# BUTSpeechFIT/huggingface_asr

Measured on AMD Instinct MI355X. Metric: audio-seconds/sec encoder fwd+CTC, E-Branchformer-base, higher is better.
Workload: dtype bf16; 1 GPU; E-Branchformer-base enc+CTC (relative-pos), 32x10s 16kHz clips/GPU: fbank+CMVN -> conv2d sub -> 16 layers -> CTC head -> CTC loss (the batch-independent projection of the relative-position table, 0.2 % of the FLOPs, is cached across steps); per_gpu_batch=32, frames=1000, encoder_frames=250, parallelism=replicas x1 (no exchange step), steps_in_flight=4, wide_tiles=True, hw_queues=8

## Files before the change

### huggingface_asr_amd/_lib.py

```python
from __future__ import annotations

import ctypes as C
import os

_HERE = os.path.dirname(os.path.abspath(__file__))
LIB_PATH = os.environ.get("HFASR_HIP_LIB") or os.path.join(_HERE, "libhfasr_hip.so")

vp, i32, i64, f32, f64, sz = C.c_void_p, C.c_int, C.c_long, C.c_float, C.c_double, C.c_size_t


class EbfConfig(C.Structure):
    _fields_ = [(n, i32) for n in ("B", "T", "F", "d", "H", "I", "L", "V", "C1", "C2", "K", "stride", "pad",
                                   "is_causal", "pos_type", "csgu_kernel", "merge_kernel", "csgu_act", "use_macaron")] + \
               [("ln_eps", f32), ("logits_f32", i32), ("logits_ld", i32), ("branch_overlap", i32), ("extra_layers", i32), ("layer_mixing", i32), ("csgu_linear", i32),
                ("context_mode", i32), ("gate_blk", i32), ("ln_fold", i32), ("wide_tiles", i32)]


class LnRedDesc(C.Structure):
    _fields_ = [("partial", vp), ("nblk", i32), ("d", i32), ("dgamma", vp), ("dbeta", vp), ("kind", i32)]


class Gpt2Config(C.Structure):
    _fields_ = [("d", i32), ("H", i32), ("L", i32), ("V", i32), ("eps", f32), ("step_form", i32), ("act", i32)]


GLOBAL_SLOTS, LAYER_SLOTS = 24, 64

SIGNATURES = {
    "mi_gemm_bf16": [vp, i64, vp, i64, vp, i32, vp, i64, i32, vp, i64, f32, i32, i32, i32, i32, i32, i32, vp],
    "mi_conv2d_cl_bf16": [vp, vp, vp, vp] + [i32] * 13 + [vp],
    "mi_gemm_bf16_v": [vp, i64, vp, i64, vp, i32, vp, i64, i32, vp, i64, f32, i32, i32, i32, i32, i32, i32, i32, vp],
    "mi_conv2d_cl_bf16_v": [vp, vp, vp, vp] + [i32] * 14 + [vp],
    "mi_conv2d_first_gelu": [vp, vp, vp, vp] + [i32] * 10 + [vp],
    "mi_conv2d_first_geo": [vp, vp, vp, vp] + [i32] * 13 + [vp],
    "mi_conv2d_first_gated_gelu": [vp, vp, vp, vp, vp, vp] + [i32] * 10 + [vp],
    "mi_conv2d_cl_geo_bf16": [vp, vp, vp, vp] + [i32] * 15 + [vp],
    "mi_gated_act_bf16": [vp, i64, vp, i64, vp, i64, i32, i32, i32, i32, i32, i32, vp],
    "mi_im2col_cl_geo_bf16": [vp, vp] + [i32] * 12 + [vp],
    "mi_col2im_cl_bf16": [vp, vp] + [i32] * 13 + [vp],
    "mi_gated_act_bwd_bf16": [vp, i64, vp, i64, vp, i64, vp, i64, vp, i64, i32, i32, i32, i32, i32, vp],
    "mi_conv2d_first_wgrad": [vp, vp, vp, vp] + [i32] * 12 + [vp, vp],
    "mi_gemm_lnfold_bf16": [vp, i64, vp, i64, vp, vp, vp, i32, f32, vp, i64, i32, i32, i32, i32, vp],
    "mi_gemm_resid_stats_f32": [vp, i64, vp, i64, vp, vp, i64, vp, i64, f32, vp, i64, vp, i32, i32, i32, vp],
    "mi_layernorm_fold": [vp, i64, vp, i32, vp, vp, f32, vp, i64, vp, i64, vp, i32, i32, vp],
    "mi_layernorm_chain": [vp, i64, vp, i32, vp, vp, f32, vp, i64, vp, vp, f32, vp, i64, vp, i64, vp, vp, vp, i64, i32, i32, vp],
    "mi_cast_f32_bf16": [vp, i64, vp, i64, i32, i32, vp],
    "mi_rotary_bf16": [vp, i64, vp, i64, vp, vp, i32, i32, i32, i32, vp],
    "mi_attention_bf16": [vp, i64, vp, i64, vp, i64, i32, vp, i64, vp, vp, vp, vp, i64, i32, i32, i32, i32, f32, i32, vp],
    "mi_attention_qkv_bf16": [vp, i64, vp, i64, vp, i64, vp, i64, vp, vp, vp, vp, i64, i32, i32, i32, i64, i32, i32, f32, i32, vp],
    "mi_attention_qkv_bf16_v": [vp, i64, vp, i64, vp, i64, vp, i64, vp, vp, vp, vp, i64, i32, i32, i32, i64, i32, i32, f32, i32, i32, vp],
    "mi_attention_x_lse_bf16": [vp, i64, vp, i64, vp, i64, vp, vp, i64, vp, i32, i32, i32, i32, i32, f32, i32, f32, C.c_uint, C.c_uint, vp],
    "mi_attention_x_bwd_probs": [vp, i64, vp, i64, vp, i64, vp, vp, i64, vp, i64, vp, vp, vp, i64, vp, i64, i32, i32, i32, i32, i32, f32, i32, f32, C.c_uint, C.c_uint, vp],
    "mi_attention_qkv_lse_bf16": [vp, i64, vp, i64, vp, i64, vp, i64, vp, vp, vp, vp, i64, vp, i32, i32, i32, i32, f32, i32, f32, C.c_uint, C.c_uint, vp],
    "mi_attention_qkv_bwd_probs": [vp, i64, vp, i64, vp, i64, vp, i64, vp, vp, vp, vp, i64, vp, i64, vp, vp, vp, i64, vp, i64, i32,
                                   vp, i64, vp, vp, vp, vp, i64, i32, i32, i32, i32, f32, i32, f32, C.c_uint, C.c_uint, i32, vp],
    "mi_attention_qkv_bwd_fused": [vp, vp, vp, i64, vp, vp, i64, vp, i64, vp, vp, vp, vp, i64, vp, sz, i32, i32, i32, i32, f32, vp],
    "mi_row_stats_bf16": [vp, i64, i32, f32, vp, i32, vp],
    "mi_csgu_bf16": [vp, i64, vp, vp, vp, vp, vp, vp, i64, i32, i32, i32, i32, i32, i32, i32, vp],
    "mi_dwconv_residual_bf16": [vp, i64, vp, vp, vp, i64, i32, i32, i32, i32, i32, vp],
    "mi_fbank_f64": [vp, i64, vp, i32, vp, vp, vp, vp, vp, vp, i32, i32, i32, f64, f64, vp],
    "mi_trim_zeros_pad_f32": [vp, i64, vp, i32, i32, i32, vp, i64, i32, vp, vp, vp, vp],
    "mi_cmvn_utterance": [vp, vp, i32, i32, i32, i32, i32, f32, vp],
    "mi_cmvn_global": [vp, i64, i32, vp, vp, vp],
    "mi_row_lse": [vp, i64, i32, i32, vp, i32, vp],
    "mi_gemm_lse_f32": [vp, i64, vp, i64, vp, vp, i64, vp, vp, i32, i32, i32, vp],
    "mi_gemm_lse_workspace_floats": [i32, i32],
    "mi_row_argmax": [vp, i64, i32, i32, vp, i32, vp],
# ... 191 lines not shown
```

### huggingface_asr_amd/csrc/encoder.hip

```cpp
#include "ebf_layout.hpp"

namespace {

struct Ws {
    bf16_t *act1, *act2, *a0, *a1, *a2, *a1r, *h, *qk, *vt, *ctx, *cat, *m2, *s, *hid;
    bf16_t *cv, *lin;
    bf16_t *z1, *g1, *z2, *g2;
    float *feo, *x, *stats, *lnst;
    float *mixed, *lh, *sw;
    int* lens;
    size_t bytes;
};

Ws carve(const mi_ebf_config& c, const Dims& d, void* base) {
    Carver k{(char*)base, 0};
    auto bf = [&](size_t n) { return (bf16_t*)k.take(n * 2); };
    auto f32 = [&](size_t n) { return (float*)k.take(n * 4); };
    Ws w;
    const size_t M = d.M, dd = c.d, I = c.I, n1 = (size_t)c.B * d.T1 * d.F1 * c.C1, n2 = (size_t)c.B * d.T2 * d.F2 * c.C2;
    w.act1 = bf(n1); w.act2 = bf(n2);
    w.z1 = w.g1 = w.z2 = w.g2 = nullptr;
    if (c.context_mode == 1) {
        if (!conv1_gated_fused(c.B, d.T1, d.F1, c.C1, c.K)) { w.z1 = bf(n1); w.g1 = bf(n1); }
        w.z2 = bf(2 * n2);
// ... 207 lines not shown
                                  w.hid, d, nullptr, 0, nullptr, nullptr, nullptr, 0, M, d, st);
    if (c.use_macaron)
        return mi_layernorm_chain(w.x, d, nullptr, T2, Lf(l, FIN_LN_G), Lf(l, FIN_LN_B), LEPS, w.x, d,
                                  Lf(l + 1, FF1_LN_G), Lf(l + 1, FF1_LN_B), LEPS, w.a0, d, nullptr, 0, nullptr, nullptr, nullptr, 0, M, d, st);
    return mi_layernorm_chain(w.x, d, nullptr, T2, Lf(l, FIN_LN_G), Lf(l, FIN_LN_B), LEPS, w.x, d,
                              Lf(l + 1, ATT_LN_G), Lf(l + 1, ATT_LN_B), LEPS, w.a1, d, nullptr, 0,
                              Lf(l + 1, MLP_LN_G), Lf(l + 1, MLP_LN_B), w.a2, d, M, d, st);
}

int Fwd::folded_layer(int l) const {
    const int gv = c.wide_tiles ? 40 : 0;
    const int npg = c.wide_tiles ? d / 64 : d / 32;
    RUN(mi_gemm_lnfold_bf16(w.a0, d, Lw(l, FF1_WF), d, Lf(l, FF1_SF), Lf(l, FF1_CF), w.lnst, 1, LEPS, w.h, I, 1, M, I, d, st));
    RUN(mi_gemm_resid_stats_f32_v(w.h, I, Lw(l, FF1_W2), I, Lf(l, FF1_B2), w.x, d, w.x, d, 0.5f, w.a0, d, w.lnst, M, d, I, gv, st));
    RUN(mi_gemm_lnfold_bf16(w.a0, d, Lw(l, QKV_WF), d, Lf(l, QKV_SF), Lf(l, QKV_CF), w.lnst, npg, LEPS, w.qk, 3 * d, 0, M, 3 * d, d, st));
    RUN(attention_qkv(l));
    RUN(mi_gemm_bf16_v(w.ctx, d, Lw(l, ATT_WO), d, Lf(l, ATT_BO), 1, w.cat, 2 * d, 0, nullptr, 0, 1.f, 0, M, d, d, 0, 0, gv, st));
    RUN(mi_gemm_lnfold_bf16(w.a0, d, Lw(l, MLP_WF), d, Lf(l, MLP_SF), Lf(l, MLP_CF), w.lnst, npg, LEPS, w.h, I, 1, M, I, d, st));
    RUN(local_gate(l, st));
    RUN(mi_gemm_bf16_v(w.s, I / 2, Lw(l, MLP_W2), I / 2, Lf(l, MLP_B2), 1, w.cat + d, 2 * d, 0, nullptr, 0, 1.f, 0, M, d, I / 2, 0, 0, gv, st));
    RUN(merge_dwconv(l));
    RUN(mi_gemm_resid_stats_f32_v(w.m2, 2 * d, Lw(l, MRG_W), 2 * d, Lf(l, MRG_B), w.x, d, w.x, d, 1.0f, w.a0, d, w.lnst, M, d, 2 * d, gv, st));
    RUN(mi_gemm_lnfold_bf16(w.a0, d, Lw(l, FF2_WF), d, Lf(l, FF2_SF), Lf(l, FF2_CF), w.lnst, npg, LEPS, w.h, I, 1, M, I, d, st));
    RUN(mi_gemm_bf16_v(w.h, I, Lw(l, FF2_W2), I, Lf(l, FF2_B2), 1, w.x, d, 1, w.x, d, 0.5f, 0, M, d, I, 0, 0, gv, st));
    if (l + 1 == c.L) return MI_OK;
    return mi_layernorm_fold(w.x, d, nullptr, T2, Lf(l, FIN_LN_G), Lf(l, FIN_LN_B), LEPS, w.x, d, w.a0, d, w.lnst, M, d, st);
}

int Fwd::encoder_exit(int l, float* last_hidden) const {
    const bool tune = c.layer_mixing || c.extra_layers;
    float* lh = (last_hidden || !tune) ? last_hidden : w.lh;
    RUN(mi_layernorm_chain(w.x, d, nullptr, T2, Lf(l, FIN_LN_G), Lf(l, FIN_LN_B), LEPS, nullptr, 0,
                           Gf(G_ENC_LN_G), Gf(G_ENC_LN_B), c.ln_eps, w.hid, d, lh, d, nullptr, nullptr, nullptr, 0, M, d, st));
    if (!tune) return MI_OK;
    const float* top = lh;
    if (c.layer_mixing) {
        RUN(mi_axpy_dev_f32(w.mixed, lh, (long)M * d, w.sw + c.L, 0, st));
        top = w.mixed;
    }
    return c.extra_layers ? enter_layer(top, c.L) : mi_add2_cast_bf16(top, d, nullptr, 0, w.hid, d, M, d, 1.f, st);
}

int Fwd::ctc_head(void* logits, float* lse, float* lse_workspace, int* best, float* amax_workspace) const {
    if (!best && !logits) return MI_OK;
    const long ldl = c.logits_ld > 0 ? c.logits_ld : c.V + 1;
    int rc = MI_ERR_UNSUPPORTED;
// ... 86 lines not shown
```

### huggingface_asr_amd/csrc/gemm_8p.hip

```cpp
#include "gemm_args.hpp"
#include <type_traits>

#ifndef GEMM_FLOOR
#define GEMM_FLOOR 0
#endif
#ifndef GEMM128_LOADER
#define GEMM128_LOADER 0
#endif

namespace {

typedef __attribute__((address_space(1))) const void* gptr_t;
typedef __attribute__((address_space(3))) void* lptr_t;

constexpr int TB = 256, BK = 64;
constexpr int BUF = 65536, BOFF = 32768;

template <int N>
__device__ __forceinline__ void wait_vm() {
    if constexpr (N >= 0) asm volatile("s_waitcnt vmcnt(%0)" ::"n"(N) : "memory");
}
__device__ __forceinline__ void barrier() {
    __builtin_amdgcn_sched_barrier(0);
    asm volatile("s_barrier" ::: "memory");
// ... 1027 lines not shown
                sm += dpp_f32<0x141, 0xF>(0.f, sm); sq += dpp_f32<0x141, 0xF>(0.f, sq);
                if ((ec & 7) == 0 && m < p.M) *reinterpret_cast<f32x2*>(p.stats_out + (long)m * LN_STATS_STRIDE + (((n0 >> 7) << 2) + (ec >> 3)) * 2) = f32x2{sm, sq};
            }
        }
    } else {
        bf16_t* C = reinterpret_cast<bf16_t*>(p.C);
#pragma unroll
        for (int u = 0; u < 8; ++u) {
            const int row = wave * 16 + u * 2 + er;
            const f32x4 v = *reinterpret_cast<const f32x4*>(smem + row * 512 + ((ec ^ (row & 31)) << 4));
            const int m = m0 + row, n = n0 + ec * 4;
            bf16x4 o = {f2bf(v.x), f2bf(v.y), f2bf(v.z), f2bf(v.w)};
            if (p.drop_p > 0.f) {
                float k4[4];
                mask_keep4(p.drop_key, ((unsigned long long)m * (unsigned)p.N + (unsigned)n) >> 2, p.drop_p, 1.f / (1.f - p.drop_p), k4);
#pragma unroll
                for (int q = 0; q < 4; ++q) o[q] = f2bf(bf2f(o[q]) * k4[q]);
            }
            if (m < p.M) *reinterpret_cast<bf16x4*>(C + (long)m * p.ldc + n) = o;
        }
    }
}

}

bool gemm_8p_supported(const GemmArgs& a, bool conv) {
    if (a.M <= 0 || a.N <= 0 || (a.K % BK) != 0 || a.K < 2 * BK) return false;
    if (a.col_T || a.bias_mode == 2) return false;
    if (a.resid && (!a.out_f32 || (a.N % TB) != 0 || ((uintptr_t)a.resid & 15) || (a.ldr % 4) != 0)) return false;
    if (((uintptr_t)a.A & 15) || ((uintptr_t)a.W & 15) || ((uintptr_t)a.C & 15) || (a.ldw % 8)) return false;
    if (a.out_f32) {
        if (conv || a.act != 0 || (a.ldc % 4) != 0 || a.ldc < ((a.N + 3) & ~3)) return false;
    } else {
        if ((a.N % TB) != 0 || (a.ldc % 8) != 0) return false;
        if (a.bias_mode == 1 && ((uintptr_t)a.bias & 15)) return false;
    }
    if (a.gated && (!conv || a.out_f32 || a.act != 1)) return false;
    if (a.ln_stats) {
        if (conv || a.out_f32 || a.gated || a.act > 1 || a.bias_mode != 1 || !a.ln_colsum || ((uintptr_t)a.ln_colsum & 15) || ((uintptr_t)a.ln_stats & 15)) return false;
        if (!(a.ln_npart == 1 || (a.ln_npart >= 4 && a.ln_npart <= 16 && (a.ln_npart % 4) == 0))) return false;
    }
    if (a.act >= 3) {
        if (conv || a.out_f32 || a.gated || a.ln_stats || a.resid || a.col_T || a.act > 4 || (a.aux_kind != 1 && a.aux_kind != 2) || a.drop_p < 0.f || a.drop_p >= 1.f) return false;
        if (a.act == 3 && (!a.aux || ((uintptr_t)a.aux & 15) || (a.ldaux % 8))) return false;
        if (a.act == 4 && (!a.C2 || ((uintptr_t)a.C2 & 15) || (a.ldc2 % 8))) return false;
    } else if (a.C2 || a.stats_out) {
// ... 52 lines not shown
    if (a.out_f32) {
        const bool attr32 = set_lds_attr(gemm8p_kernel<false, 0, true>, 2 * BUF);
        (void)attr32;
        launch_dense(PF_8P_OUT32, gemm8p_kernel<false, 0, true>, dim3(grid), dim3(512), (size_t)2 * BUF, stream, a);
        return MI_OK;
    }
    if (a.ln_stats) {
        const bool attr_l = set_lds_attr(gemm8p_kernel<false, 0, false, false, true>, 2 * BUF + 2048) && set_lds_attr(gemm8p_kernel<false, 1, false, false, true>, 2 * BUF + 2048);
        (void)attr_l;
        if (a.act) launch_dense(PF_8P_GELU, gemm8p_kernel<false, 1, false, false, true>, dim3(grid), dim3(512), (size_t)2 * BUF + 2048, stream, a);
        else launch_dense(PF_8P, gemm8p_kernel<false, 0, false, false, true>, dim3(grid), dim3(512), (size_t)2 * BUF + 2048, stream, a);
        return MI_OK;
    }
    if (a.gated) {
        const bool attr_g = set_lds_attr(gemm8p_kernel<true, 1, false, true>, 2 * BUF);
        (void)attr_g;
        launch_dense(PF_8P_CONV, gemm8p_kernel<true, 1, false, true>, dim3(grid), dim3(512), (size_t)2 * BUF, stream, a);
        return MI_OK;
    }
    launch_dense(conv ? PF_8P_CONV : (a.act ? PF_8P_GELU : PF_8P), kerns[conv ? 1 : 0][a.act], dim3(grid), dim3(512), (size_t)2 * BUF, stream, a);
    return MI_OK;
}

bool gemm_8p128_supported(const GemmArgs& a) {
    if (a.M <= 0 || a.N <= 0 || (a.N % 128) != 0 || (a.K % BK) != 0 || a.K < 5 * BK) return false;
    if (a.col_T || a.bias_mode == 2) return false;
    if (a.resid && !a.out_f32) return false;
    if (((uintptr_t)a.A & 15) || ((uintptr_t)a.W & 15) || ((uintptr_t)a.C & 15) || (a.lda % 8) || (a.ldw % 8)) return false;
    if (a.out_f32 ? (a.ldc % 4) != 0 : (a.ldc % 8) != 0) return false;
    if (a.resid && (((uintptr_t)a.resid & 15) || (a.ldr % 4) != 0)) return false;
    if (a.bias_mode == 1 && ((uintptr_t)a.bias & 15)) return false;
    if ((long)a.M * a.lda * 2 >= (1l << 32) || (long)a.N * a.ldw * 2 >= (1l << 32)) return false;
    if (a.ln_stats) return false;
    if ((a.C2 || a.stats_out) && (!a.out_f32 || a.N > 512 || (a.K % 128) != 0 || (a.C2 && (((uintptr_t)a.C2 & 7) || (a.ldc2 % 4))) || ((uintptr_t)a.stats_out & 7))) return false;
    return true;
}

int gemm_8p128_launch(const GemmArgs& a, int ring, hipStream_t stream) {
    const bool attr_set = set_lds_attr(gemm8p128_kernel<4>, 4 * B128_BUF);
    (void)attr_set;
    const int grid = cdiv(a.M, 128) * (a.N / 128);
    if (ring == 0) ring = (GEMM128_LOADER == 1 && a.K >= 2048) ? 2 : 3;
    if (ring == 2) {
        const bool attr_l = set_lds_attr(gemm8p128l_kernel, 4 * B128_BUF);
        (void)attr_l;
        launch_dense(PF_8P128, gemm8p128l_kernel, dim3(grid), dim3(512), (size_t)4 * B128_BUF, stream, a);
// ... 12 lines not shown
```

### huggingface_asr_amd/csrc/gemm_args.hpp

```cpp
#pragma once
#include "common.hpp"
#include <hip/hip_ext.h>

struct GemmArgs {
    const bf16_t* A; long lda;
    const bf16_t* W; long ldw;
    const float* bias; int bias_mode;
    void* C; long ldc; int out_f32;
    const float* resid; long ldr; float alpha;
    int act;
    int col_T, col_Tp;
    int M, N, K;
    int variant;
    int Tin, Fin, Cin, Tout, Fout, KW, stride, pad_t, pad_f;
    int stride_f;
    int gated;
    const float* ln_stats; int ln_npart; const float* ln_colsum; float ln_eps;
    bf16_t* C2; long ldc2; float* stats_out;
    const bf16_t* aux; long ldaux; int aux_kind; float drop_p; unsigned long long drop_key;
    float* lse_part; int lse_ld;
    float* amax_part; int amax_ld;
    int ce; const long* ce_labels; float* ce_target; const float* ce_lse; const float* ce_g;
};
constexpr int LN_STATS_STRIDE = 32;

bool gemm_glds_supported(const GemmArgs& a, bool conv);
int gemm_glds_launch(const GemmArgs& a, bool conv, hipStream_t stream);


bool gemm_8p_supported(const GemmArgs& a, bool conv);
int gemm_8p_launch(const GemmArgs& a, bool conv, hipStream_t stream);
bool gemm_8p128_supported(const GemmArgs& a);
int gemm_8p128_launch(const GemmArgs& a, int ring, hipStream_t stream);


extern "C" int mi_profile_take_events(hipEvent_t* start, hipEvent_t* stop, int family);
enum { PF_8P = 0, PF_8P_GELU = 1, PF_8P_CONV = 2, PF_8P_OUT32 = 3, PF_8P128 = 4, PF_GLDS = 5, PF_GENERIC = 6, PF_8P_AMAX = 7, PF_8P_CE = 8, PF_COUNT = 9 };

template <typename F, typename... Args>
inline void launch_dense(int family, F kernel, dim3 grid, dim3 block, size_t lds, hipStream_t stream, Args... args) {
    hipEvent_t e0, e1;
    if (mi_profile_take_events(&e0, &e1, family)) hipExtLaunchKernelGGL(kernel, grid, block, (std::uint32_t)lds, stream, e0, e1, 0, args...);
    else hipLaunchKernelGGL(kernel, grid, block, lds, stream, args...);
}
```

### huggingface_asr_amd/csrc/gemm_bf16.hip

```cpp
#include "gemm_args.hpp"

namespace {

constexpr int BM = 128, BN = 128, BK = 64;
constexpr int NT = 256;

__device__ __forceinline__ int swz(int row, int chunk) { return chunk ^ ((row >> 1) & 7); }

template <bool CONV>
__global__ __launch_bounds__(NT) void gemm_bf16_kernel(GemmArgs p) {
    extern __shared__ __attribute__((aligned(16))) char smem[];
    bf16_t* sA = reinterpret_cast<bf16_t*>(smem);
    bf16_t* sB = sA + 2 * BM * BK;

    const int tid = threadIdx.x;
    const int lane = tid & 63, wave = tid >> 6;
    const int wm = wave >> 1, wn = wave & 1;

    const int ntm = (p.M + BM - 1) / BM, ntn = (p.N + BN - 1) / BN;
    const int nwg = ntm * ntn;
    int bid = blockIdx.x;
    {
        const int q = nwg >> 3, r = nwg & 7, xcd = bid & 7, idx = bid >> 3;
        bid = (xcd < r ? xcd * (q + 1) : r * (q + 1) + (xcd - r) * q) + idx;
// ... 293 lines not shown
                                         void* C2, long ldc2, float* stats_out, int M, int N, int K, int variant, hipStream_t stream);
extern "C" int mi_gemm_resid_stats_f32(const void* A, long lda, const void* W, long ldw, const float* bias, float* C, long ldc, const float* resid, long ldr, float alpha,
                                       void* C2, long ldc2, float* stats_out, int M, int N, int K, hipStream_t stream) {
    return mi_gemm_resid_stats_f32_v(A, lda, W, ldw, bias, C, ldc, resid, ldr, alpha, C2, ldc2, stats_out, M, N, K, 0, stream);
}
extern "C" int mi_gemm_resid_stats_f32_v(const void* A, long lda, const void* W, long ldw, const float* bias, float* C, long ldc, const float* resid, long ldr, float alpha,
                                         void* C2, long ldc2, float* stats_out, int M, int N, int K, int variant, hipStream_t stream) {
    MI_ENTER();
    GemmArgs a{};
    a.A = (const bf16_t*)A; a.lda = lda; a.W = (const bf16_t*)W; a.ldw = ldw; a.bias = bias; a.bias_mode = bias ? 1 : 0;
    a.C = C; a.ldc = ldc; a.out_f32 = 1; a.resid = resid; a.ldr = ldr; a.alpha = alpha; a.act = 0; a.M = M; a.N = N; a.K = K;
    a.C2 = (bf16_t*)C2; a.ldc2 = ldc2; a.stats_out = stats_out;
    if (!A || !W || !C || !resid || (variant != 0 && variant != 40 && variant != 42 && variant != 43)) return MI_ERR_ARG;
    const bool wide = variant == 40;
    if (wide ? !gemm_8p_supported(a, false) : !gemm_8p128_supported(a)) return MI_ERR_UNSUPPORTED;
    const int slot = mi_profile_hook_begin(stream, 2.0 * M * N * K);
    const int rc = wide ? gemm_8p_launch(a, false, stream) : gemm_8p128_launch(a, variant == 42 ? 3 : (variant == 43 ? 2 : 0), stream);
    if (slot >= 0) mi_profile_hook_end(slot, stream);
    if (rc != MI_OK) return rc;
    MI_CHECK_LAUNCH();
    return MI_OK;
}

namespace {
__global__ __launch_bounds__(256) void lse_merge_kernel(const float* __restrict__ part, int ld, int npair, float* __restrict__ lse, int M) {
    const int g = threadIdx.x & 15;
    const int row = blockIdx.x * 16 + (threadIdx.x >> 4);
    const float* pr = part + (long)min(row, M - 1) * ld;
    float mx = -INFINITY;
    for (int t = g; t < npair; t += 16) mx = fmaxf(mx, pr[2 * t]);
    mx = fmaxf(mx, dpp_f32<0xB1, 0xF>(mx, mx)); mx = fmaxf(mx, dpp_f32<0x4E, 0xF>(mx, mx));
    mx = fmaxf(mx, dpp_f32<0x141, 0xF>(mx, mx)); mx = fmaxf(mx, dpp_f32<0x140, 0xF>(mx, mx));
    float s = 0.f;
    for (int t = g; t < npair; t += 16) {
        const f32x2 q = *reinterpret_cast<const f32x2*>(pr + 2 * t);
        if (q.x > -INFINITY) s += q.y * __expf(q.x - mx);
    }
    s += dpp_f32<0xB1, 0xF>(0.f, s); s += dpp_f32<0x4E, 0xF>(0.f, s);
    s += dpp_f32<0x141, 0xF>(0.f, s); s += dpp_f32<0x140, 0xF>(0.f, s);
    if (g == 0 && row < M) lse[row] = mx + __logf(s);
}
}

extern "C" size_t mi_gemm_lse_workspace_floats(int M, int N) { return (size_t)(M > 0 ? M : 0) * 8 * (size_t)((N + 255) / 256); }

extern "C" int mi_gemm_lse_f32(const void* A, long lda, const void* W, long ldw, const float* bias, float* C, long ldc, float* lse, float* workspace,
// ... 129 lines not shown
```

### huggingface_asr_amd/ops.py

```python
from __future__ import annotations

import math

import torch

from . import _lib

BF16 = torch.bfloat16


def _p(t):
    return 0 if t is None else t.data_ptr()


_PINNED_STREAM = None


def _stream():
    return torch.cuda.current_stream().cuda_stream if _PINNED_STREAM is None else _PINNED_STREAM


class pinned_stream:

    def __enter__(self):
# ... 105 lines not shown
    _lib.check(_lib.lib().mi_gated_act_bf16(z2.data_ptr(), z2.stride(0), g2.data_ptr(), g2.stride(0), out.data_ptr(), out.stride(0), B, T, Fq, C, share, blk, _stream()),
               "mi_gated_act_bf16")
    return out


def gemm_lnfold(xb, wf, colsum, cbias, stats, npart, eps=1e-5, act="none", out=None):
    M, K = xb.shape
    N = wf.shape[0]
    if out is None:
        out = torch.empty((M, N), device=xb.device, dtype=BF16)
    _lib.check(_lib.lib().mi_gemm_lnfold_bf16(xb.data_ptr(), xb.stride(0), wf.data_ptr(), wf.stride(0), colsum.data_ptr(), cbias.data_ptr(), stats.data_ptr(), int(npart), float(eps),
                                              out.data_ptr(), out.stride(0), {"none": 0, "gelu": 1}[act], M, N, K, _stream()), "mi_gemm_lnfold_bf16")
    return out


def gemm_resid_stats(a, w, bias, resid, alpha=1.0, wide=False, variant=None):
    M, K = a.shape
    N = w.shape[0]
    c = torch.empty((M, N), device=a.device, dtype=torch.float32)
    c2 = torch.empty((M, N), device=a.device, dtype=BF16)
    st = torch.zeros((M, 32), device=a.device, dtype=torch.float32)
    _lib.check(_lib.lib().mi_gemm_resid_stats_f32_v(a.data_ptr(), a.stride(0), w.data_ptr(), w.stride(0), _p(bias), c.data_ptr(), c.stride(0), _p(resid), resid.stride(0) if resid is not None else 0,
                                                    float(alpha), c2.data_ptr(), c2.stride(0), st.data_ptr(), M, N, K, (40 if wide else 0) if variant is None else int(variant), _stream()), "mi_gemm_resid_stats_f32_v")
    return c, c2, st


def layernorm_fold(x, ln=None, eps=1e-5, lengths=None, T=1):
    M, d = x.shape
    g, b = ln if ln else (None, None)
    y = torch.empty_like(x)
    yb = torch.empty((M, d), device=x.device, dtype=BF16)
    st = torch.zeros((M, 32), device=x.device, dtype=torch.float32)
    _lib.check(_lib.lib().mi_layernorm_fold(x.data_ptr(), x.stride(0), _p(lengths), T, _p(g), _p(b), float(eps), y.data_ptr(), y.stride(0), yb.data_ptr(), yb.stride(0), st.data_ptr(),
                                            M, d, _stream()), "mi_layernorm_fold")
    return y, yb, st


def layernorm_chain(x, *, lengths=None, T=1, ln1=None, eps1=1e-5, store_y=None, lna=None, eps2=1e-5, outa=None,
                    outa32=None, lnb=None, outb=None):
    M, d = x.shape
    g1, b1 = ln1 if ln1 else (None, None)
    ga, ba = lna if lna else (None, None)
    gb, bb = lnb if lnb else (None, None)
    rc = _lib.lib().mi_layernorm_chain(x.data_ptr(), x.stride(0), _p(lengths), T, _p(g1), _p(b1), eps1,
                                       _p(store_y), store_y.stride(0) if store_y is not None else 0,
                                       _p(ga), _p(ba), eps2, _p(outa), outa.stride(0) if outa is not None else 0,
# ... 562 lines not shown
```

### include/hfasr_hip.h

```cpp
#ifndef HFASR_HIP_H
#define HFASR_HIP_H
#include <stddef.h>
#include <stdint.h>

#ifdef __cplusplus
extern "C" {
#endif

typedef struct ihipStream_t* mi_stream_t;

const char* mi_last_error(void);

int mi_profile_create(int capacity);
void mi_profile_enable(int on);
void mi_profile_reset(void);
int mi_profile_count(void);
int mi_profile_summary(double* total_ms, double* total_flops);
int mi_profile_calibrate(mi_stream_t stream, int n, double* median_ms);
int mi_profile_summary_family(int family, double* total_ms, double* total_flops, int* launches);

int mi_gemm_bf16(const void* A, long lda, const void* W, long ldw, const float* bias, int bias_mode,
                 void* C, long ldc, int out_f32, const float* resid, long ldr, float alpha, int act,
                 int M, int N, int K, int col_T, int col_Tp, mi_stream_t stream);
int mi_gemm_bf16_v(const void* A, long lda, const void* W, long ldw, const float* bias, int bias_mode,
// ... 13 lines not shown

int mi_conv2d_first_geo(const float* x, const float* w, const float* bias, void* out_cl_bf16, int B, int T, int F, int C,
                        int KH, int KW, int stride_t, int stride_f, int pad_t, int pad_f, int T1, int F1, int act, mi_stream_t stream);
int mi_conv2d_first_gated_gelu(const float* x, const float* w, const float* bias, const float* gw, const float* gbias, void* out_cl_bf16,
                               int B, int T, int F, int C, int K, int stride, int pad_t, int pad_f, int T1, int F1, mi_stream_t stream);
int mi_conv2d_cl_geo_bf16(const void* in, const void* weight, const float* bias, void* out, int B, int Tin, int Fin, int Cin, int Cout, int KH, int KW,
                          int stride_t, int stride_f, int pad_t, int pad_f, int Tout, int Fout, int act, int gated, mi_stream_t stream);
int mi_gated_act_bf16(const void* z, long ldz, const void* g, long ldg, void* out, long ldo, int B, int T, int Fq, int C, int share, int blk, mi_stream_t stream);

int mi_gemm_dropout_bf16(const void* A, long lda, const void* W, long ldw, const float* bias, void* C, long ldc, int out_f32, const float* resid, long ldr,
                         float alpha, float drop_p, unsigned seed, unsigned stream_id, int M, int N, int K, mi_stream_t stream);
int mi_gemm_act_fwd_bf16(const void* A, long lda, const void* W, long ldw, const float* bias, void* pre, long ldp, void* h, long ldh, int kind,
                         float drop_p, unsigned seed, unsigned stream_id, int M, int N, int K, mi_stream_t stream);
int mi_gemm_act_bwd_bf16(const void* dY, long ldy, const void* Wt, long ldw, const void* pre, long ldp, void* dX, long ldx, int kind,
                         float drop_p, unsigned seed, unsigned stream_id, int M, int N, int K, mi_stream_t stream);
int mi_gemm_lnfold_bf16(const void* xb, long lda, const void* Wf, long ldw, const float* colsum, const float* cbias, const float* stats, int npart, float eps,
                        void* C, long ldc, int act, int M, int N, int K, mi_stream_t stream);
int mi_gemm_resid_stats_f32(const void* A, long lda, const void* W, long ldw, const float* bias, float* C, long ldc, const float* resid, long ldr, float alpha,
                            void* C2, long ldc2, float* stats_out, int M, int N, int K, mi_stream_t stream);
int mi_gemm_resid_stats_f32_v(const void* A, long lda, const void* W, long ldw, const float* bias, float* C, long ldc, const float* resid, long ldr, float alpha,
                              void* C2, long ldc2, float* stats_out, int M, int N, int K, int variant, mi_stream_t stream);
int mi_layernorm_fold(const float* x, long ldx, const int* lengths, int T, const float* g1, const float* b1, float eps1, float* y32, long ldy,
                      void* yb_bf16, long ldyb, float* stats, int M, int d, mi_stream_t stream);

int mi_layernorm_chain(const float* x, long ldx, const int* lengths, int T,
                       const float* g1, const float* b1, float eps1, float* y32, long ldy,
                       const float* ga, const float* ba, float eps2, void* outa_bf16, long lda,
                       float* outa_f32, long lda32,
                       const float* gb, const float* bb, void* outb_bf16, long ldb,
                       int M, int d, mi_stream_t stream);

int mi_cast_f32_bf16(const float* x, long ldx, void* out, long ldo, int M, int d, mi_stream_t stream);

int mi_rotary_bf16(const void* x, long ldx, void* out, long ldo, const float* cos_t, const float* sin_t,
                   int M, int T, int H, int hd, mi_stream_t stream);

int mi_attention_bf16(const void* q, long ldq, const void* k, long ldk, const void* vt, long ldvt, int Tp,
                      const void* pos, long ldp, const float* bias_u, const float* bias_v,
                      const int* lengths, void* out, long ldo, int B, int T, int H, int hd,
                      float scale, int causal, mi_stream_t stream);

int mi_attention_qkv_bf16(const void* q, long ldq, const void* k, long ldk, const void* v, long ldv,
                          const void* pos, long ldp, const float* bias_u, const float* bias_v,
                          const int* lengths, void* out, long ldo, int B, int T, int Tk, long kv_bstride, int H, int hd,
                          float scale, int causal, mi_stream_t stream);
int mi_attention_qkv_bf16_v(const void* q, long ldq, const void* k, long ldk, const void* v, long ldv,
// ... 366 lines not shown
```

Measured before the change: 82680 audio-seconds/sec.

## Fuse FF2 down-projection, residual add and final LayerNorm into one row-complete GEMM

Adds a new GEMM kernel in which each 128-row block computes the full 512-wide output row. This lets the epilogue add the residual and apply the per-layer final LayerNorm in-block, then write the fp32 activations, the bf16 copy and the row stats. In wide-tile mode the encoder uses it for the FF2 down-projection of every non-last layer. That removes the separate layernorm_fold launch and the extra round trip of the residual stream through memory. The trade-off is a large LDS footprint and only M/128 blocks (about 63 for this batch), which may underfill the GPU compared with the previous tiled GEMM.

```diff
diff --git a/huggingface_asr_amd/_lib.py b/huggingface_asr_amd/_lib.py
--- a/huggingface_asr_amd/_lib.py
+++ b/huggingface_asr_amd/_lib.py
@@ -43,6 +43,8 @@
     "mi_gemm_lnfold_bf16": [vp, i64, vp, i64, vp, vp, vp, i32, f32, vp, i64, i32, i32, i32, i32, vp],
     "mi_gemm_resid_stats_f32": [vp, i64, vp, i64, vp, vp, i64, vp, i64, f32, vp, i64, vp, i32, i32, i32, vp],
     "mi_layernorm_fold": [vp, i64, vp, i32, vp, vp, f32, vp, i64, vp, i64, vp, i32, i32, vp],
+    "mi_gemm_resid_ln_f32": [vp, i64, vp, i64, vp, vp, i64, vp, i64, f32, vp, vp, f32, vp, i64, vp, i32, i32, i32, vp],
+    "mi_gemm_resid_ln_launches": [i32],
     "mi_layernorm_chain": [vp, i64, vp, i32, vp, vp, f32, vp, i64, vp, vp, f32, vp, i64, vp, i64, vp, vp, vp, i64, i32, i32, vp],
     "mi_cast_f32_bf16": [vp, i64, vp, i64, i32, i32, vp],
     "mi_rotary_bf16": [vp, i64, vp, i64, vp, vp, i32, i32, i32, i32, vp],
diff --git a/huggingface_asr_amd/csrc/encoder.hip b/huggingface_asr_amd/csrc/encoder.hip
--- a/huggingface_asr_amd/csrc/encoder.hip
+++ b/huggingface_asr_amd/csrc/encoder.hip
@@ -253,6 +253,10 @@
     RUN(merge_dwconv(l));
     RUN(mi_gemm_resid_stats_f32_v(w.m2, 2 * d, Lw(l, MRG_W), 2 * d, Lf(l, MRG_B), w.x, d, w.x, d, 1.0f, w.a0, d, w.lnst, M, d, 2 * d, gv, st));
     RUN(mi_gemm_lnfold_bf16(w.a0, d, Lw(l, FF2_WF), d, Lf(l, FF2_SF), Lf(l, FF2_CF), w.lnst, npg, LEPS, w.h, I, 1, M, I, d, st));
+    if (c.wide_tiles && l + 1 < c.L) {
+        const int rc = mi_gemm_resid_ln_f32(w.h, I, Lw(l, FF2_W2), I, Lf(l, FF2_B2), w.x, d, w.x, d, 0.5f, Lf(l, FIN_LN_G), Lf(l, FIN_LN_B), LEPS, w.a0, d, w.lnst, M, d, I, st);
+        if (rc != MI_ERR_UNSUPPORTED) return rc;
+    }
     RUN(mi_gemm_bf16_v(w.h, I, Lw(l, FF2_W2), I, Lf(l, FF2_B2), 1, w.x, d, 1, w.x, d, 0.5f, 0, M, d, I, 0, 0, gv, st));
     if (l + 1 == c.L) return MI_OK;
     return mi_layernorm_fold(w.x, d, nullptr, T2, Lf(l, FIN_LN_G), Lf(l, FIN_LN_B), LEPS, w.x, d, w.a0, d, w.lnst, M, d, st);
diff --git a/huggingface_asr_amd/csrc/gemm_8p.hip b/huggingface_asr_amd/csrc/gemm_8p.hip
--- a/huggingface_asr_amd/csrc/gemm_8p.hip
+++ b/huggingface_asr_amd/csrc/gemm_8p.hip
@@ -1073,6 +1073,242 @@
     }
 }
 
+constexpr int ROW_BUF = 81920, ROW_WOFF = 16384;
+constexpr int ROW_EPI = 131072;
+constexpr int ROW_LDS = 2 * ROW_BUF;
+
+__global__ __launch_bounds__(512, 2) void gemm8prow_kernel(GemmArgs p) {
+    extern __shared__ __attribute__((aligned(16))) char smem[];
+    const int tid = threadIdx.x, lane = tid & 63;
+    const int wave = __builtin_amdgcn_readfirstlane(tid >> 6);
+    const int wr = wave >> 2, wc = wave & 3;
+    const int m0 = blockIdx.x * 128;
+
+    const char* Ab = reinterpret_cast<const char*>(p.A);
+    const char* Wb = reinterpret_cast<const char*>(p.W);
+    unsigned offA[2], offW[8];
+    {
+        const int prow = lane >> 3, pc = lane & 7;
+#pragma unroll
+        for (int e = 0; e < 2; ++e) {
+            const int r = (2 * wave + e) * 8 + prow;
+            offA[e] = (unsigned)min(m0 + r, p.M - 1) * (unsigned)(p.lda * 2) + (unsigned)((pc ^ ((r >> 1) & 7)) * 16);
+        }
+#pragma unroll
+        for (int e = 0; e < 8; ++e) {
+            const int r = (8 * wave + e) * 8 + prow;
+            offW[e] = (unsigned)r * (unsigned)(p.ldw * 2) + (unsigned)((pc ^ ((r >> 1) & 7)) * 16);
+        }
+    }
+    auto stage = [&](int kt, unsigned buf) {
+#pragma unroll
+        for (int e = 0; e < 2; ++e)
+            __builtin_amdgcn_global_load_lds((gptr_t)(Ab + offA[e] + (unsigned)kt * 128u), (lptr_t)(smem + buf + (2 * wave + e) * 1024), 16, 0, 0);
+#pragma unroll
+        for (int e = 0; e < 8; ++e)
+            __builtin_amdgcn_global_load_lds((gptr_t)(Wb + offW[e] + (unsigned)kt * 128u), (lptr_t)(smem + buf + ROW_WOFF + (8 * wave + e) * 1024), 16, 0, 0);
+    };
+    const int fr = lane & 15, fq = lane >> 4;
+    const unsigned low = fr * 128 + ((fq ^ ((fr >> 1) & 7)) << 4);
+    const unsigned aRd = wr * 64 * 128 + low, bRd = ROW_WOFF + wc * 64 * 128 + low;
+
+    f32x4 acc[4][8];
+#pragma unroll
+    for (int i = 0; i < 4; ++i)
+#pragma unroll
+        for (int j = 0; j < 8; ++j) acc[i][j] = f32x4{0.f, 0.f, 0.f, 0.f};
+    bf16x8 fa[4], fb[8];
+    auto sub = [&](int kt, unsigned cb, auto S, auto DO_STAGE, auto WAIT) {
+        constexpr unsigned ks = decltype(S)::value * 64u;
+#pragma unroll
+        for (int j = 0; j < 8; ++j) fb[j] = *reinterpret_cast<const bf16x8*>(smem + cb + (bRd ^ ks) + ((j >> 2) * 256 + (j & 3) * 16) * 128);
+#pragma unroll
+        for (int i = 0; i < 4; ++i) fa[i] = *reinterpret_cast<const bf16x8*>(smem + cb + (aRd ^ ks) + i * 16 * 128);
+        if constexpr (decltype(DO_STAGE)::value) stage(kt + 1, ROW_BUF - cb);
+        wait_vm<decltype(WAIT)::value>();
+        wait_lds();
+        barrier();
+        __builtin_amdgcn_s_setprio(1);
+#pragma unroll
+        for (int i = 0; i < 4; ++i)
+#pragma unroll
+            for (int j = 0; j < 8; ++j)
+                acc[i][j] = __builtin_amdgcn_mfma_f32_16x16x32_bf16(fb[j], fa[i], acc[i][j], 0, 0, 0);
+        __builtin_amdgcn_s_setprio(0);
+        barrier();
+    };
+    using T = std::true_type;
+    using F = std::false_type;
+    using I0 = std::integral_constant<int, 0>;
+    using I1 = std::integral_constant<int, 1>;
+    using NOWAIT = std::integral_constant<int, -1>;
+    const int nk = p.K / BK;
+    stage(0, 0);
+    wait_vm<0>();
+    barrier();
+    if (wr == 1) barrier();
+    unsigned cb = 0;
+    int kt = 0;
+    for (; kt < nk - 1; ++kt) {
+        sub(kt, cb, I0{}, T{}, NOWAIT{});
+        sub(kt, cb, I1{}, F{}, I0{});
+        cb = ROW_BUF - cb;
+    }
+    sub(kt, cb, I0{}, F{}, NOWAIT{});
+    sub(kt, cb, I1{}, F{}, NOWAIT{});
+    if (wr == 0) barrier();
+
+    char* reg = smem + wave * 16384;
+    int el = lane;
+    asm volatile("" : "+v"(el));
+    const int r16 = el >> 4, c16 = el & 15;
+    const int cl = wc * 64 + c16 * 4;
+#pragma unroll
+    for (int j = 0; j < 8; ++j) {
+        f32x4 bj = f32x4{0.f, 0.f, 0.f, 0.f};
+        if (p.bias_mode == 1) bj = *reinterpret_cast<const f32x4*>(p.bias + (j >> 2) * 256 + wc * 64 + (j & 3) * 16 + r16 * 4);
+#pragma unroll
+        for (int i = 0; i < 4; ++i) acc[i][j] += bj;
+    }
+    const bool ln = p.rl_gamma != nullptr;
+    auto row16 = [](float x) {
+        x += dpp_f32<0xB1, 0xF>(0.f, x);
+        x += dpp_f32<0x4E, 0xF>(0.f, x);
+        x += dpp_f32<0x141, 0xF>(0.f, x);
+        x += dpp_f32<0x140, 0xF>(0.f, x);
+        return x;
+    };
+    auto rows4 = [](float r0, float r1, float r2, float r3) {
+#pragma clang fp contract(off)
+        return (r3 + r2) + (r1 + r0);
+    };
+    auto sum8 = [](f32x4 a, f32x4 b) {
+#pragma clang fp contract(off)
+        return (0.f + (((a.x + a.y) + a.z) + a.w)) + (((b.x + b.y) + b.z) + b.w);
+    };
+    auto csq4 = [](f32x4 a, float mean) {
+#pragma clang fp contract(off)
+        const float x = a.x - mean, y = a.y - mean, z = a.z - mean, w = a.w - mean;
+        return __builtin_fmaf(w, w, __builtin_fmaf(z, z, __builtin_fmaf(x, x, y * y)));
+    };
+    auto norm4 = [](f32x4 a, float mean, float rstd, f32x4 g, f32x4 b) {
+#pragma clang fp contract(off)
+        const float x = (a.x - mean) * rstd, y = (a.y - mean) * rstd, z = (a.z - mean) * rstd, w = (a.w - mean) * rstd;
+        return f32x4{__builtin_fmaf(x, g.x, b.x), __builtin_fmaf(y, g.y, b.y), __builtin_fmaf(z, g.z, b.z), __builtin_fmaf(w, g.w, b.w)};
+    };
+    auto pair8 = [](f32x4 a, f32x4 b, float& sm, float& sq) {
+#pragma clang fp contract(off)
+        sm = (0.f + ((a.x + a.y) + (a.z + a.w))) + ((b.x + b.y) + (b.z + b.w));
+        sq = (__builtin_fmaf(a.x, a.x, a.y * a.y) + __builtin_fmaf(a.z, a.z, a.w * a.w)) + (__builtin_fmaf(b.x, b.x, b.y * b.y) + __builtin_fmaf(b.z, b.z, b.w * b.w));
+    };
+    float* C = reinterpret_cast<float*>(p.C);
+#pragma unroll
+    for (int qt = 0; qt < 4; ++qt) {
+#pragma unroll
+        for (int j = 0; j < 8; ++j) *reinterpret_cast<f32x4*>(reg + c16 * 512 + (((j * 4 + r16) ^ c16) << 4)) = acc[qt][j];
+        f32x4 v[4][2];
+#pragma unroll
+        for (int u = 0; u < 4; ++u) {
+            const int m = min(m0 + wr * 64 + qt * 16 + u * 4 + r16, p.M - 1);
+#pragma unroll
+            for (int h = 0; h < 2; ++h) v[u][h] = *reinterpret_cast<const f32x4*>(p.resid + ((unsigned)m * (unsigned)p.ldr + (unsigned)(cl + h * 256)));
+        }
+        asm volatile("s_waitcnt lgkmcnt(0)" ::: "memory");
+#pragma unroll
+        for (int u = 0; u < 4; ++u) {
+            const int row = u * 4 + r16;
+#pragma unroll
+            for (int h = 0; h < 2; ++h) {
+                const f32x4 t = *reinterpret_cast<const f32x4*>(reg + row * 512 + (((h * 16 + c16) ^ row) << 4));
+                v[u][h] = v[u][h] + p.alpha * t;
+            }
+        }
+        char* tab = smem + ROW_EPI + qt * 2048;
+        const int rl = wr * 16 + r16;
+        if (ln) {
+            float mean[4], rstd[4];
+#pragma unroll
+            for (int u = 0; u < 4; ++u) {
+                const float s = row16(sum8(v[u][0], v[u][1]));
+                if (c16 == 0) *reinterpret_cast<float*>(tab + ((rl + u * 4) * 4 + wc) * 4) = s;
+                __builtin_amdgcn_sched_barrier(0);
+            }
+            asm volatile("s_waitcnt lgkmcnt(0)" ::: "memory");
+            barrier();
+#pragma unroll
+            for (int u = 0; u < 4; ++u) {
+                const f32x4 t = *reinterpret_cast<const f32x4*>(tab + (rl + u * 4) * 16);
+                mean[u] = rows4(t.x, t.y, t.z, t.w) / 512.f;
+            }
+#pragma unroll
+            for (int u = 0; u < 4; ++u) {
+                const float q = row16(csq4(v[u][0], mean[u]) + csq4(v[u][1], mean[u]));
+                if (c16 == 0) *reinterpret_cast<float*>(tab + 512 + ((rl + u * 4) * 4 + wc) * 4) = q;
+                __builtin_amdgcn_sched_barrier(0);
+            }
+            f32x4 g4[2], b4[2];
+#pragma unroll
+            for (int h = 0; h < 2; ++h) {
+                g4[h] = *reinterpret_cast<const f32x4*>(p.rl_gamma + cl + h * 256);
+                b4[h] = *reinterpret_cast<const f32x4*>(p.rl_beta + cl + h * 256);
+            }
+            asm volatile("s_waitcnt lgkmcnt(0)" ::: "memory");
+            barrier();
+#pragma unroll
+            for (int u = 0; u < 4; ++u) {
+                const f32x4 t = *reinterpret_cast<const f32x4*>(tab + 512 + (rl + u * 4) * 16);
+                rstd[u] = rsqrtf(rows4(t.x, t.y, t.z, t.w) / 512.f + p.ln_eps);
+            }
+#pragma unroll
+            for (int u = 0; u < 4; ++u) {
+#pragma unroll
+                for (int h = 0; h < 2; ++h) v[u][h] = norm4(v[u][h], mean[u], rstd[u], g4[h], b4[h]);
+                __builtin_amdgcn_sched_barrier(0);
+            }
+        }
+#pragma unroll
+        for (int u = 0; u < 4; ++u) {
+            const int m = m0 + wr * 64 + qt * 16 + u * 4 + r16;
+            if (m < p.M) {
+#pragma unroll
+                for (int h = 0; h < 2; ++h) {
+                    const f32x4 y = v[u][h];
+                    *reinterpret_cast<f32x4*>(C + ((unsigned)m * (unsigned)p.ldc + (unsigned)(cl + h * 256))) = y;
+                    *reinterpret_cast<bf16x4*>(p.C2 + ((unsigned)m * (unsigned)p.ldc2 + (unsigned)(cl + h * 256))) = bf16x4{f2bf(y.x), f2bf(y.y), f2bf(y.z), f2bf(y.w)};
+                }
+            }
+            float sm, sq;
+            pair8(v[u][0], v[u][1], sm, sq);
+            sm = row16(sm); sq = row16(sq);
+            if (c16 == 0) *reinterpret_cast<f32x2*>(tab + 1024 + ((rl + u * 4) * 4 + wc) * 8) = f32x2{sm, sq};
+            __builtin_amdgcn_sched_barrier(0);
+        }
+        asm volatile("s_waitcnt lgkmcnt(0)" ::: "memory");
+        barrier();
+        if (wc == 0 && c16 == 0) {
+#pragma unroll
+            for (int u = 0; u < 4; ++u) {
+                const int m = m0 + wr * 64 + qt * 16 + u * 4 + r16;
+                const f32x4 t0 = *reinterpret_cast<const f32x4*>(tab + 1024 + (rl + u * 4) * 32), t1 = *reinterpret_cast<const f32x4*>(tab + 1024 + (rl + u * 4) * 32 + 16);
+                if (m < p.M) *reinterpret_cast<f32x2*>(p.stats_out + (long)m * LN_STATS_STRIDE) = f32x2{rows4(t0.x, t0.z, t1.x, t1.z), rows4(t0.y, t0.w, t1.y, t1.w)};
+            }
+        }
+    }
+}
+
+}
+
+bool gemm_8prow_supported(const GemmArgs& a) {
+    if (a.M <= 0 || a.N != 512 || (a.K % BK) != 0 || a.K < 2 * BK) return false;
+    if (!a.out_f32 || !a.resid || !a.C2 || !a.stats_out || a.act != 0 || a.col_T || a.bias_mode == 2 || a.ln_stats || a.drop_p != 0.f) return false;
+    if (((uintptr_t)a.A & 15) || ((uintptr_t)a.W & 15) || (a.lda % 8) || (a.ldw % 8) || a.lda < a.K || a.ldw < a.K) return false;
+    if (((uintptr_t)a.C & 15) || (a.ldc % 4) || a.ldc < 512 || ((uintptr_t)a.resid & 15) || (a.ldr % 4) || a.ldr < 512) return false;
+    if (((uintptr_t)a.C2 & 7) || (a.ldc2 % 4) || a.ldc2 < 512 || ((uintptr_t)a.stats_out & 7)) return false;
+    if (a.bias_mode == 1 && ((uintptr_t)a.bias & 15)) return false;
+    if ((a.rl_gamma != nullptr) != (a.rl_beta != nullptr) || ((uintptr_t)a.rl_gamma & 15) || ((uintptr_t)a.rl_beta & 15)) return false;
+    if ((long)a.M * a.lda * 2 >= (1l << 32) || (long)a.N * a.ldw * 2 >= (1l << 32)) return false;
+    if ((long)a.M * a.ldc >= (1l << 32) || (long)a.M * a.ldr >= (1l << 32) || (long)a.M * a.ldc2 >= (1l << 32)) return false;
+    return true;
 }
 
 bool gemm_8p_supported(const GemmArgs& a, bool conv) {
@@ -1171,6 +1407,12 @@
     return MI_OK;
 }
 
+int gemm_8prow_launch(const GemmArgs& a, hipStream_t stream) {
+    if (!set_lds_attr(gemm8prow_kernel, ROW_LDS)) return MI_ERR_LAUNCH;
+    launch_dense(PF_8P128, gemm8prow_kernel, dim3(cdiv(a.M, 128)), dim3(512), (size_t)ROW_LDS, stream, a);
+    return MI_OK;
+}
+
 bool gemm_8p128_supported(const GemmArgs& a) {
     if (a.M <= 0 || a.N <= 0 || (a.N % 128) != 0 || (a.K % BK) != 0 || a.K < 5 * BK) return false;
     if (a.col_T || a.bias_mode == 2) return false;
diff --git a/huggingface_asr_amd/csrc/gemm_args.hpp b/huggingface_asr_amd/csrc/gemm_args.hpp
--- a/huggingface_asr_amd/csrc/gemm_args.hpp
+++ b/huggingface_asr_amd/csrc/gemm_args.hpp
@@ -21,6 +21,7 @@
     float* lse_part; int lse_ld;
     float* amax_part; int amax_ld;
     int ce; const long* ce_labels; float* ce_target; const float* ce_lse; const float* ce_g;
+    const float* rl_gamma; const float* rl_beta;
 };
 constexpr int LN_STATS_STRIDE = 32;
 
@@ -32,6 +33,8 @@
 int gemm_8p_launch(const GemmArgs& a, bool conv, hipStream_t stream);
 bool gemm_8p128_supported(const GemmArgs& a);
 int gemm_8p128_launch(const GemmArgs& a, int ring, hipStream_t stream);
+bool gemm_8prow_supported(const GemmArgs& a);
+int gemm_8prow_launch(const GemmArgs& a, hipStream_t stream);
 
 
 extern "C" int mi_profile_take_events(hipEvent_t* start, hipEvent_t* stop, int family);
diff --git a/huggingface_asr_amd/csrc/gemm_bf16.hip b/huggingface_asr_amd/csrc/gemm_bf16.hip
--- a/huggingface_asr_amd/csrc/gemm_bf16.hip
+++ b/huggingface_asr_amd/csrc/gemm_bf16.hip
@@ -1,4 +1,5 @@
 #include "gemm_args.hpp"
+#include <atomic>
 
 namespace {
 
@@ -339,6 +340,28 @@
     return MI_OK;
 }
 
+static std::atomic<int> g_resid_ln_launches{0};
+extern "C" int mi_gemm_resid_ln_launches(int reset) {
+    return reset ? g_resid_ln_launches.exchange(0) : g_resid_ln_launches.load();
+}
+extern "C" int mi_gemm_resid_ln_f32(const void* A, long lda, const void* W, long ldw, const float* bias, float* C, long ldc, const float* resid, long ldr, float alpha,
+                                    const float* gamma, const float* beta, float eps, void* C2, long ldc2, float* stats_out, int M, int N, int K, hipStream_t stream) {
+    MI_ENTER();
+    GemmArgs a{};
+    a.A = (const bf16_t*)A; a.lda = lda; a.W = (const bf16_t*)W; a.ldw = ldw; a.bias = bias; a.bias_mode = bias ? 1 : 0;
+    a.C = C; a.ldc = ldc; a.out_f32 = 1; a.resid = resid; a.ldr = ldr; a.alpha = alpha; a.act = 0; a.M = M; a.N = N; a.K = K;
+    a.C2 = (bf16_t*)C2; a.ldc2 = ldc2; a.stats_out = stats_out; a.rl_gamma = gamma; a.rl_beta = beta; a.ln_eps = eps;
+    if (!A || !W || !C || !resid || !C2 || !stats_out || (gamma != nullptr) != (beta != nullptr)) return MI_ERR_ARG;
+    if (!gemm_8prow_supported(a)) return MI_ERR_UNSUPPORTED;
+    const int slot = mi_profile_hook_begin(stream, 2.0 * M * N * K);
+    const int rc = gemm_8prow_launch(a, stream);
+    if (slot >= 0) mi_profile_hook_end(slot, stream);
+    if (rc != MI_OK) return rc;
+    MI_CHECK_LAUNCH();
+    g_resid_ln_launches.fetch_add(1);
+    return MI_OK;
+}
+
 namespace {
 __global__ __launch_bounds__(256) void lse_merge_kernel(const float* __restrict__ part, int ld, int npair, float* __restrict__ lse, int M) {
     const int g = threadIdx.x & 15;
diff --git a/huggingface_asr_amd/ops.py b/huggingface_asr_amd/ops.py
--- a/huggingface_asr_amd/ops.py
+++ b/huggingface_asr_amd/ops.py
@@ -151,6 +151,18 @@
     st = torch.zeros((M, 32), device=a.device, dtype=torch.float32)
     _lib.check(_lib.lib().mi_gemm_resid_stats_f32_v(a.data_ptr(), a.stride(0), w.data_ptr(), w.stride(0), _p(bias), c.data_ptr(), c.stride(0), _p(resid), resid.stride(0) if resid is not None else 0,
                                                     float(alpha), c2.data_ptr(), c2.stride(0), st.data_ptr(), M, N, K, (40 if wide else 0) if variant is None else int(variant), _stream()), "mi_gemm_resid_stats_f32_v")
+    return c, c2, st
+
+
+def gemm_resid_ln(a, w, bias, resid, alpha=1.0, ln=None, eps=1e-5, out=None, out_bf16=None, stats=None):
+    M, K = a.shape
+    N = w.shape[0]
+    g, b = ln if ln else (None, None)
+    c = torch.empty((M, N), device=a.device, dtype=torch.float32) if out is None else out
+    c2 = torch.empty((M, N), device=a.device, dtype=BF16) if out_bf16 is None else out_bf16
+    st = torch.zeros((M, 32), device=a.device, dtype=torch.float32) if stats is None else stats
+    _lib.check(_lib.lib().mi_gemm_resid_ln_f32(a.data_ptr(), a.stride(0), w.data_ptr(), w.stride(0), _p(bias), c.data_ptr(), c.stride(0), resid.data_ptr(), resid.stride(0), float(alpha),
+                                               _p(g), _p(b), float(eps), c2.data_ptr(), c2.stride(0), st.data_ptr(), M, N, K, _stream()), "mi_gemm_resid_ln_f32")
     return c, c2, st
 
 
diff --git a/include/hfasr_hip.h b/include/hfasr_hip.h
--- a/include/hfasr_hip.h
+++ b/include/hfasr_hip.h
@@ -59,6 +59,9 @@
                               void* C2, long ldc2, float* stats_out, int M, int N, int K, int variant, mi_stream_t stream);
 int mi_layernorm_fold(const float* x, long ldx, const int* lengths, int T, const float* g1, const float* b1, float eps1, float* y32, long ldy,
                       void* yb_bf16, long ldyb, float* stats, int M, int d, mi_stream_t stream);
+int mi_gemm_resid_ln_f32(const void* A, long lda, const void* W, long ldw, const float* bias, float* C, long ldc, const float* resid, long ldr, float alpha,
+                         const float* gamma, const float* beta, float eps, void* C2, long ldc2, float* stats_out, int M, int N, int K, mi_stream_t stream);
+int mi_gemm_resid_ln_launches(int reset);
 
 int mi_layernorm_chain(const float* x, long ldx, const int* lengths, int T,
                        const float* g1, const float* b1, float eps1, float* y32, long ldy,
```

Result: slower. 81570 audio-seconds/sec (-1.3%).
